# saber/ORB_SLAM2_Annotate

Measured on AMD Instinct MI355X. Metric: ORB extract+match frames/sec (kp/desc/matches bit-exact vs CPU oracle on the checked frames of every run), higher is better.
Workload: dtype u8; 1 GPU; KITTI 00 stereo 1241x376 nFeatures=2000: extract L+R + ComputeStereoMatches (synthetic stereo pairs; frames/s counts STEREO frames = 2 images each)

## Files before the change

orb_slam2_annotate_amd/csrc/k_match.hip:

```cpp
#include "kernels.h"
#include "match_kernels.h"

namespace orbfe {

namespace {
struct Desc { uint32_t w[8]; };

__device__ __forceinline__ Desc load_desc(const uint8_t* base, uint32_t idx) {
  const uint4* p = reinterpret_cast<const uint4*>(base + (size_t)idx * 32);
  const uint4 a = p[0], b = p[1];
  Desc d;
  d.w[0] = a.x; d.w[1] = a.y; d.w[2] = a.z; d.w[3] = a.w;
  d.w[4] = b.x; d.w[5] = b.y; d.w[6] = b.z; d.w[7] = b.w;
  return d;
}
__device__ __forceinline__ int hdist(const Desc& a, const Desc& b) {
  int d = 0;
#pragma unroll
  for (int i = 0; i < 8; i++) d += __popc(a.w[i] ^ b.w[i]);
  return d;
}
__device__ __forceinline__ uint32_t wave_min_u32(uint32_t v) { return wave_min_u32_dpp(v); }
__device__ __forceinline__ int rot_bin(float a1, float a2) {
  const float factor = 1.0f / 30;
// ... 236 lines not shown
    if (a.hasMp2[idx2]) continue;
    const bool st2 = a.stereo2[idx2] != 0;
    if (a.onlyStereo && !st2) continue;
    const uint32_t dist = (uint32_t)hdist(d1, load_desc(a.desc2, idx2));
    if (dist > 50u) continue;
    const float x2 = a.x2[idx2], y2 = a.y2[idx2];
    const int oc = a.octave2[idx2];
    if (!st1 && !st2) {
      const float dex = __fsub_rn(a.ex, x2), dey = __fsub_rn(a.ey, y2);
      if (__fadd_rn(__fmul_rn(dex, dex), __fmul_rn(dey, dey)) < __fmul_rn(100.0f, a.scaleFactors2[oc])) continue;
    }
    const float num = __fadd_rn(__fadd_rn(__fmul_rn(la, x2), __fmul_rn(lb, y2)), lc);
    if (den == 0) continue;
    const float dsqr = __fdiv_rn(__fmul_rn(num, num), den);
    if (!((double)dsqr < __dmul_rn(3.84, (double)a.levelSigma2_2[oc]))) continue;
    const uint32_t key = (dist << 16) | (0xffffu - (uint32_t)p);
    best = key < best ? key : best;
  }
  best = wave_min_u32(best);
  if (lane == 0) {
    if (best != 0xffffffffu) {
      const uint32_t pos = 0xffffu - (best & 0xffffu);
      const uint32_t idx2 = a.indices2[tq.off2 + pos];
      a.match[idx1] = (int32_t)idx2;
      a.bin[idx1] = (int8_t)rot_bin(a.angle1[idx1], a.angle2[idx2]);
    }
  }
}

__global__ __launch_bounds__(256) void k_search_triangulation(TriArgs a) {
  search_triangulation_one(a, blockIdx.x * 4 + (threadIdx.x >> 6), threadIdx.x & 63);
}
__global__ __launch_bounds__(256) void k_search_triangulation_multi(const TriArgs* __restrict__ args, const int32_t* __restrict__ blockStart,
                                                                    int K) {
  const int g = blockIdx.x;
  int lo = 0, hi = K;
  while (hi - lo > 1) {
    const int mid = (lo + hi) >> 1;
    if (blockStart[mid] <= g) lo = mid; else hi = mid;
  }
  const TriArgs a = args[lo];
  search_triangulation_one(a, (g - blockStart[lo]) * 4 + (threadIdx.x >> 6), threadIdx.x & 63);
}

__global__ __launch_bounds__(256) void k_rot_prune(int32_t* __restrict__ match, const int8_t* __restrict__ bin,
                                                   int n, int checkOri, int32_t* __restrict__ nMatches,
                                                   int batchStride) {
  match += (size_t)blockIdx.x * batchStride;
  bin += (size_t)blockIdx.x * batchStride;
  nMatches += blockIdx.x;
  __shared__ int hist[30];
  __shared__ int keep[3];
  __shared__ int total;
  const int tid = threadIdx.x;
  if (tid < 30) hist[tid] = 0;
  if (tid == 0) total = 0;
  __syncthreads();
  int mine = 0;
  for (int i = tid; i < n; i += 256)
    if (match[i] >= 0) { mine++; atomicAdd(&hist[bin[i]], 1); }
  if (mine) atomicAdd(&total, mine);
  __syncthreads();
  if (!checkOri) { if (tid == 0) *nMatches = total; return; }
  if (tid == 0) {
    int max1 = 0, max2 = 0, max3 = 0, i1 = -1, i2 = -1, i3 = -1;
    for (int i = 0; i < 30; i++) {
      const int s = hist[i];
      if (s > max1) { max3 = max2; max2 = max1; max1 = s; i3 = i2; i2 = i1; i1 = i; }
      else if (s > max2) { max3 = max2; max2 = s; i3 = i2; i2 = i; }
      else if (s > max3) { max3 = s; i3 = i; }
    }
    if ((float)max2 < __fmul_rn(0.1f, (float)max1)) { i2 = -1; i3 = -1; }
    else if ((float)max3 < __fmul_rn(0.1f, (float)max1)) { i3 = -1; }
    keep[0] = i1; keep[1] = i2; keep[2] = i3;
    int kept = 0;
    for (int i = 0; i < 30; i++)
      if (i == i1 || i == i2 || i == i3) kept += hist[i];
    *nMatches = kept;
  }
  __syncthreads();
  const int k0 = keep[0], k1 = keep[1], k2 = keep[2];
  for (int i = tid; i < n; i += 256)
    if (match[i] >= 0) {
      const int b = bin[i];
      if (b != k0 && b != k1 && b != k2) match[i] = -1;
    }
}

void launch_search_by_bow(hipStream_t s, const BowArgs& a, int nPairs, int maxCnt2) {
  if (nPairs <= 0) return;
  const size_t lds = (size_t)((maxCnt2 + 15) & ~15);
  if (maxCnt2 <= 64) hipLaunchKernelGGL((k_search_by_bow<1>), dim3(nPairs), dim3(64), lds, s, a);
  else if (maxCnt2 <= 128) hipLaunchKernelGGL((k_search_by_bow<2>), dim3(nPairs), dim3(64), lds, s, a);
  else hipLaunchKernelGGL((k_search_by_bow<4>), dim3(nPairs), dim3(64), lds, s, a);
}
void launch_search_by_bow_multi(hipStream_t s, const BowArgs* d_args, const int32_t* d_pairStart, int K, int nPairsTotal, int maxCnt2) {
  if (nPairsTotal <= 0 || K <= 0) return;
  const size_t lds = (size_t)((maxCnt2 + 15) & ~15);
  if (maxCnt2 <= 64) hipLaunchKernelGGL((k_search_by_bow_multi<1>), dim3(nPairsTotal), dim3(64), lds, s, d_args, d_pairStart, K);
  else if (maxCnt2 <= 128) hipLaunchKernelGGL((k_search_by_bow_multi<2>), dim3(nPairsTotal), dim3(64), lds, s, d_args, d_pairStart, K);
  else hipLaunchKernelGGL((k_search_by_bow_multi<4>), dim3(nPairsTotal), dim3(64), lds, s, d_args, d_pairStart, K);
}
void launch_search_triangulation(hipStream_t s, const TriArgs& a) {
  if (a.nQueries <= 0) return;
  hipLaunchKernelGGL(k_search_triangulation, dim3((a.nQueries + 3) / 4), dim3(256), 0, s, a);
}
void launch_search_triangulation_multi(hipStream_t s, const TriArgs* d_args, const int32_t* d_blockStart, int K, int totalBlocks) {
  if (K <= 0 || totalBlocks <= 0) return;
  hipLaunchKernelGGL(k_search_triangulation_multi, dim3(totalBlocks), dim3(256), 0, s, d_args, d_blockStart, K);
}
void launch_rot_prune(hipStream_t s, int32_t* match, const int8_t* bin, int n, int checkOri, int32_t* nMatches) {
  hipLaunchKernelGGL(k_rot_prune, dim3(1), dim3(256), 0, s, match, bin, n, checkOri, nMatches, 0);
}
void launch_rot_prune_batch(hipStream_t s, int32_t* match, const int8_t* bin, int n, int nArrays, int checkOri, int32_t* nMatches) {
  if (nArrays <= 0) return;
  hipLaunchKernelGGL(k_rot_prune, dim3(nArrays), dim3(256), 0, s, match, bin, n, checkOri, nMatches, n);
}
void launch_search_by_bow_batch(hipStream_t s, const BowBatch& b, int nPairs, int checkOri, int32_t* d_nMatches, int maxNodes) {
  if (nPairs <= 0 || b.capacity <= 0) return;
  const size_t lds = (size_t)((b.capacity + 15) & ~15);
  const int gx = (maxNodes > 0 && maxNodes < b.capacity) ? maxNodes : b.capacity;
  hipLaunchKernelGGL(k_search_by_bow_batch, dim3(gx, nPairs), dim3(64), lds, s, b);
  hipLaunchKernelGGL(k_rot_prune, dim3(nPairs), dim3(256), 0, s, b.match, b.bin, b.capacity, checkOri, d_nMatches,
                     b.capacity);
}

struct StereoPair {
  const float* kpL; const uint8_t* descL; int N;
  const float* kpR; const uint8_t* descR; int Nr;
  int frameL, frameR;
  float* uRight; float* depth; int32_t* sad;
  const int32_t* rowStart; const int32_t* sortedIdx; const float4* sortedRec;
};

__device__ __forceinline__ uint32_t row16_min_u32(uint32_t v) {
  uint32_t t;
  t = (uint32_t)__builtin_amdgcn_update_dpp((int)v, (int)v, 0x121, 0xf, 0xf, false); v = t < v ? t : v;
  t = (uint32_t)__builtin_amdgcn_update_dpp((int)v, (int)v, 0x122, 0xf, 0xf, false); v = t < v ? t : v;
  t = (uint32_t)__builtin_amdgcn_update_dpp((int)v, (int)v, 0x124, 0xf, 0xf, false); v = t < v ? t : v;
  t = (uint32_t)__builtin_amdgcn_update_dpp((int)v, (int)v, 0x128, 0xf, 0xf, false); v = t < v ? t : v;
  return v;
}
__device__ __forceinline__ int row16_sum_i32(int v) {
  v += __builtin_amdgcn_update_dpp(0, v, 0x121, 0xf, 0xf, false);
  v += __builtin_amdgcn_update_dpp(0, v, 0x122, 0xf, 0xf, false);
  v += __builtin_amdgcn_update_dpp(0, v, 0x124, 0xf, 0xf, false);
  v += __builtin_amdgcn_update_dpp(0, v, 0x128, 0xf, 0xf, false);
  return v;
}
constexpr uint32_t selpair(int o) { return (uint32_t)o | 0x0c00u | ((uint32_t)(o + 1) << 16) | 0x0c000000u; }

struct StereoLds { LevelView L[kMaxLevels], R[kMaxLevels]; float scale[2 * kMaxLevels]; };

template <bool kRec>
__device__ __forceinline__ void stereo_row16(const StereoArgs& a, const StereoLds& lv, const StereoPair& pp, int iL, bool alive,
                                             int lane) {
  const int sub = lane & 15, rowBase = lane & 48;
  float uL = 0.f, vL = 0.f;
  int levelL = 0;
  bool record = true;
  if (alive) {
    const float* kl = pp.kpL + (size_t)iL * 7;
    uL = kl[0]; vL = kl[1];
    levelL = reinterpret_cast<const int32_t*>(kl)[5];
    if ((unsigned)levelL >= (unsigned)a.pyrL.nlevels || !(fabsf(uL) < 3.0e38f) || !(fabsf(vL) < 3.0e38f)) { record = false; levelL = 0; uL = vL = 0.f; }
  }
  const int row = (int)vL;
  const float minU = __fsub_rn(uL, a.maxD), maxU = uL;
  bool live = alive && record && !(maxU < 0) && row >= 0 && row < a.rows;
  int pBeg = 0, pEnd = live ? pp.Nr : 0;
  if (pp.rowStart && live) {
    int band = a.bandR;
    {
      const int oMax = levelL + 1 < a.pyrL.nlevels ? levelL + 1 : a.pyrL.nlevels - 1;
      const int bl = (int)ceilf(__fmul_rn(2.0f, lv.scale[oMax < 0 ? 0 : oMax])) + 2;
      band = bl < band ? bl : band;
    }
    int lo = row - band, hi = row + band;
    lo = lo < 0 ? 0 : lo;
    hi = hi > a.rows - 1 ? a.rows - 1 : hi;
    if (lo > hi) { live = false; pEnd = 0; }
    else { pBeg = pp.rowStart[lo]; pEnd = pp.rowStart[hi + 1]; }
  }
  Desc dL = {};
  if (live) dL = load_desc(pp.descL, iL);
  uint32_t best = 0xffffffffu;
  float bestU = 0.f;
  for (int p = pBeg + sub; __any(p < pEnd); p += 16) {
    if (p < pEnd) {
      int iR, octR;
      float yR, uR;
      if (kRec) {
        const float4 rc = pp.sortedRec[p];
        uR = rc.x; yR = rc.y; octR = __float_as_int(rc.z); iR = __float_as_int(rc.w);
      } else {
        iR = pp.rowStart ? pp.sortedIdx[p] : p;
        const float* kr = pp.kpR + (size_t)iR * 7;
        octR = reinterpret_cast<const int32_t*>(kr)[5];
        yR = kr[1];
        uR = kr[0];
      }
      if ((unsigned)octR >= (unsigned)a.pyrL.nlevels || !(fabsf(yR) < 3.0e38f)) continue;
      const float r = __fmul_rn(2.0f, lv.scale[octR]);
      const int maxr = (int)ceilf(__fadd_rn(yR, r));
      const int minr = (int)floorf(__fsub_rn(yR, r));
      const bool cand = row >= minr && row <= maxr && octR >= levelL - 1 && octR <= levelL + 1 && uR >= minU && uR <= maxU;
      if (cand) {
        const uint32_t dist = (uint32_t)hdist(dL, load_desc(pp.descR, iR));
        const uint32_t key = (dist << 20) | (uint32_t)iR;
        if (dist < 100u && key < best) { best = key; bestU = uR; }
      }
    }
  }
  const uint32_t mine = best;
  best = row16_min_u32(best);
  live = live && best != 0xffffffffu && (int)(best >> 20) < 75;
  const unsigned long long win = __ballot(mine == best);
  const uint32_t winRow = (uint32_t)(win >> rowBase) & 0xffffu;
  const int src = rowBase + (winRow ? __builtin_ctz(winRow) : 0);
  const float uR0 = __shfl(bestU, src, 64);
  float oU = -1.0f, oD = -1.0f;
  int oS = -1;
  if (__builtin_amdgcn_ballot_w64(live) != 0ull) {
  const float sf = lv.scale[kMaxLevels + levelL];
  const float scaleduL = roundf(__fmul_rn(uL, sf));
  const float scaledvL = roundf(__fmul_rn(vL, sf));
  const float scaleduR0 = roundf(__fmul_rn(uR0, sf));
  const LevelView L = lv.L[levelL], R = lv.R[levelL];
  const float iniu = scaleduR0 + 5 - 5;
  const float endu = scaleduR0 + 5 + 5 + 1;
  if (iniu < 0 || endu >= (float)R.w) live = false;
  const int cy = (int)scaledvL, cxL = (int)scaleduL, cxR0 = (int)scaleduR0;
  if (cy < 5 || cy + 5 >= L.h || cy + 5 >= R.h || cxL < 5 || cxL + 5 >= L.w || cxR0 < 10) live = false;
  uint32_t ql[4] = {0u, 0u, 0u, 0u}, qr[6] = {0u, 0u, 0u, 0u, 0u, 0u};
  if (live && sub < 11) {
    const uint8_t* pl = L.base + (size_t)pp.frameL * L.frameStride + (ptrdiff_t)(cy + sub - 5) * L.pitch + (cxL - 5);
    const uint8_t* pr = R.base + (size_t)pp.frameR * R.frameStride + (ptrdiff_t)(cy + sub - 5) * R.pitch + (cxR0 - 10);
    struct __attribute__((packed, aligned(1))) U4u { uint32_t x, y, z, w; };
    struct __attribute__((packed, aligned(1))) U2u { uint32_t x, y; };
    const bool wide = cxL >= 5 && cxL + 10 < L.w && cxR0 >= 10 && cxR0 + 13 < R.w && cy >= 5 && cy + 5 < L.h && cy + 5 < R.h;
    if (wide) {
      const U4u a4 = *reinterpret_cast<const U4u*>(pl);
      const U4u b4 = *reinterpret_cast<const U4u*>(pr);
      const U2u c2 = *reinterpret_cast<const U2u*>(pr + 16);
      ql[0] = a4.x; ql[1] = a4.y; ql[2] = a4.z;
      qr[0] = b4.x; qr[1] = b4.y; qr[2] = b4.z; qr[3] = b4.w; qr[4] = c2.x; qr[5] = c2.y;
    } else {
#pragma unroll
      for (int k = 0; k < 11; k++) ql[k >> 2] |= (uint32_t)pl[k] << (8 * (k & 3));
#pragma unroll
      for (int k = 0; k < 21; k++) qr[k >> 2] |= (uint32_t)pr[k] << (8 * (k & 3));
    }
  }
  const uint32_t cL = ((uint32_t)__shfl((int)ql[1], rowBase + 5, 64) >> 8) & 0xffu;
  const uint32_t c1 = (uint32_t)__shfl((int)qr[1], rowBase + 5, 64), c2 = (uint32_t)__shfl((int)qr[2], rowBase + 5, 64),
                 c3 = (uint32_t)__shfl((int)qr[3], rowBase + 5, 64);
  const uint32_t cLL = cL | (cL << 16);
  uint32_t A[5], B[19], C[11];
#pragma unroll
  for (int m = 0; m < 5; m++) A[m] = __builtin_amdgcn_perm(ql[(m >> 1) + 1], ql[m >> 1], selpair((2 * m) & 3));
  const uint32_t l10 = (ql[2] >> 16) & 0xffu;
#pragma unroll
  for (int t = 0; t < 19; t++) B[t] = __builtin_amdgcn_perm(qr[(t >> 2) + 1], qr[t >> 2], selpair(t & 3)) + cLL;
#pragma unroll
  for (int t = 10; t < 21; t++) C[t - 10] = ((qr[t >> 2] >> (8 * (t & 3))) & 0xffu) + cL;
  int dists[11];
#pragma unroll
  for (int s = 0; s < 11; s++) {
    const int cb = 5 + s;
    const uint32_t cw = cb < 8 ? c1 : (cb < 12 ? c2 : c3);
    const uint32_t cR = (cw >> (8 * (cb & 3))) & 0xffu;
    const uint32_t cRR = cR | (cR << 16);
    uint32_t acc = 0;
#pragma unroll
    for (int m = 0; m < 5; m++) acc = __builtin_amdgcn_sad_u16(A[m] + cRR, B[2 * m + s], acc);
    acc = __builtin_amdgcn_sad_u16(l10 + cR, C[s], acc);
    dists[s] = row16_sum_i32(sub < 11 ? (int)acc : 0);
  }
  int bestSad = 0x7fffffff, bestinc = 0;
#pragma unroll
  for (int i = 0; i < 11; i++)
    if (dists[i] < bestSad) { bestSad = dists[i]; bestinc = i - 5; }
  if (bestinc == -5 || bestinc == 5) live = false;
  float d1 = 0, d2 = 0, d3 = 0;
#pragma unroll
  for (int i = 1; i < 10; i++)
    if (i == bestinc + 5) { d1 = (float)dists[i - 1]; d2 = (float)dists[i]; d3 = (float)dists[i + 1]; }
  const float deltaR = __fdiv_rn(__fsub_rn(d1, d3),
                                 __fmul_rn(2.0f, __fsub_rn(__fadd_rn(d1, d3), __fmul_rn(2.0f, d2))));
  if (deltaR < -1 || deltaR > 1) live = false;
  float bestuR = __fmul_rn(lv.scale[levelL], __fadd_rn(__fadd_rn(scaleduR0, (float)bestinc), deltaR));
  float disparity = __fsub_rn(uL, bestuR);
  if (live && disparity >= 0 && disparity < a.maxD) {
    if (disparity <= 0) {
      disparity = 0.01f;
      bestuR = (float)__dsub_rn((double)uL, 0.01);
    }
    oD = __fdiv_rn(a.mbf, disparity);
    oU = bestuR;
    oS = bestSad;
  }
  }
  if (alive && sub == 0) { pp.uRight[iL] = oU; pp.depth[iL] = oD; pp.sad[iL] = oS; }
}

__global__ __launch_bounds__(256) void k_stereo_bucket(const float* __restrict__ kpBase, const int32_t* __restrict__ nArr,
                                                       int nFixed, int capacity, int rows,
                                                       int32_t* __restrict__ rowStartBase,
                                                       int32_t* __restrict__ sortedBase, float4* __restrict__ recBase) {
  extern __shared__ int cnt[];
  __shared__ int waveTot[4];
  ORBFE_LATENCY_KERNEL_PRIO();
  const int tid = threadIdx.x, lane = tid & 63, wave = tid >> 6, p = blockIdx.x;
  const float* kpR = nArr ? kpBase + (size_t)(2 * p + 1) * capacity * 7 : kpBase;
  int Nr = nArr ? nArr[2 * p + 1] : nFixed;
  if (Nr > capacity) Nr = capacity;
  int32_t* rowStart = rowStartBase + (size_t)p * (rows + 1);
  int32_t* sorted = sortedBase + (size_t)p * capacity;
  float4* rec = recBase ? recBase + (size_t)p * capacity : nullptr;
  for (int i = tid; i <= rows; i += 256) cnt[i] = 0;
  __syncthreads();
  for (int i = tid; i < Nr; i += 256) {
    int b = (int)floorf(kpR[(size_t)i * 7 + 1]);
    b = b < 0 ? 0 : (b > rows - 1 ? rows - 1 : b);
    atomicAdd(&cnt[b], 1);
  }
  __syncthreads();
  int run = 0;
  for (int base = 0; base <= rows; base += 256) {
    const int i = base + tid;
    const int v = i <= rows ? cnt[i] : 0;
    int x = v;
#pragma unroll
    for (int o = 1; o < 64; o <<= 1) {
      const int y = __shfl_up(x, o, 64);
      if (lane >= o) x += y;
    }
    if (lane == 63) waveTot[wave] = x;
    __syncthreads();
    int b = run;
    for (int w = 0; w < wave; w++) b += waveTot[w];
    run += waveTot[0] + waveTot[1] + waveTot[2] + waveTot[3];
    if (i <= rows) { cnt[i] = b + x - v; rowStart[i] = b + x - v; }
    __syncthreads();
  }
  for (int i = tid; i < Nr; i += 256) {
    int b = (int)floorf(kpR[(size_t)i * 7 + 1]);
    b = b < 0 ? 0 : (b > rows - 1 ? rows - 1 : b);
    const int pos = atomicAdd(&cnt[b], 1);
    sorted[pos] = i;
    if (rec) rec[pos] = make_float4(kpR[(size_t)i * 7], kpR[(size_t)i * 7 + 1], __int_as_float(reinterpret_cast<const int32_t*>(kpR)[(size_t)i * 7 + 5]),
                                    __int_as_float(i));
  }
}

__device__ __forceinline__ void stereo_stage_views(const StereoArgs& a, StereoLds& lv) {
  const int t = threadIdx.x;
  if (t < kMaxLevels) lv.L[t] = a.pyrL.lv[t];
  else if (t < 2 * kMaxLevels) lv.R[t - kMaxLevels] = a.pyrR.lv[t - kMaxLevels];
  else if (t < 4 * kMaxLevels) lv.scale[t - 2 * kMaxLevels] = a.scaleTab[t - 2 * kMaxLevels];
  __syncthreads();
}

__global__ __launch_bounds__(256) void k_stereo_match(StereoArgs a) {
  __shared__ StereoLds lv;
  stereo_stage_views(a, lv);
  const int lane = threadIdx.x & 63;
  const int iL = blockIdx.x * 16 + (threadIdx.x >> 4);
  StereoPair pp = {a.kpL, a.descL, a.N, a.kpR, a.descR, a.Nr, a.frameL, a.frameR, a.uRight, a.depth, a.sad,
                   a.rowStart, a.sortedIdx, a.rowStart ? a.sortedRec : nullptr};
  if (pp.sortedRec) stereo_row16<true>(a, lv, pp, iL, iL < a.N, lane);
  else stereo_row16<false>(a, lv, pp, iL, iL < a.N, lane);
}

__global__ __launch_bounds__(256) void k_stereo_match_batch(const StereoArgs a, const StereoBatch b) {
  ORBFE_LATENCY_KERNEL_PRIO();
  __shared__ StereoLds lv;
  stereo_stage_views(a, lv);
  const int lane = threadIdx.x & 63;
  const int iL = blockIdx.x * 16 + (threadIdx.x >> 4);
  const int p = blockIdx.y;
  int N = b.n[2 * p], Nr = b.n[2 * p + 1];
  if (N > b.capacity) N = b.capacity;
  if (Nr > b.capacity) Nr = b.capacity;
  const size_t oL = (size_t)(2 * p) * b.capacity, oR = (size_t)(2 * p + 1) * b.capacity, oO = (size_t)p * b.capacity;
  if (iL < b.capacity && iL >= N && (lane & 15) == 0) {
    b.uRight[oO + iL] = -1.0f; b.depth[oO + iL] = -1.0f; b.sad[oO + iL] = -1;
  }
  if (blockIdx.x * 16 >= N) return;
  StereoPair pp;
  pp.kpL = b.kp + oL * 7; pp.descL = b.desc + oL * 32; pp.N = N;
  pp.kpR = b.kp + oR * 7; pp.descR = b.desc + oR * 32; pp.Nr = Nr;
  pp.frameL = 2 * p; pp.frameR = 2 * p + 1;
  pp.uRight = b.uRight + oO; pp.depth = b.depth + oO; pp.sad = b.sad + oO;
  pp.rowStart = a.rowStart ? a.rowStart + (size_t)p * (a.rows + 1) : nullptr;
  pp.sortedIdx = a.rowStart ? a.sortedIdx + (size_t)p * b.capacity : nullptr;
  pp.sortedRec = (a.rowStart && a.sortedRec) ? a.sortedRec + (size_t)p * b.capacity : nullptr;
  if (pp.sortedRec) stereo_row16<true>(a, lv, pp, iL, iL < N, lane);
  else stereo_row16<false>(a, lv, pp, iL, iL < N, lane);
}

__global__ __launch_bounds__(256) void k_stereo_median_cut(int N, const int32_t* __restrict__ sad,
                                                           float* __restrict__ uRight, float* __restrict__ depth,
                                                           int32_t* __restrict__ nStereo, int pairStride) {
  sad += (size_t)blockIdx.x * pairStride;
  uRight += (size_t)blockIdx.x * pairStride;
  depth += (size_t)blockIdx.x * pairStride;
  nStereo += blockIdx.x;
  __shared__ int hist[256];
  __shared__ int sel[3];
  __shared__ int waveTot[4];
  ORBFE_LATENCY_KERNEL_PRIO();
  const int tid = threadIdx.x;
  hist[tid] = 0;
  if (tid == 0) sel[2] = 0;
  __syncthreads();
  int mine = 0;
  for (int i = tid; i < N; i += 256) {
    const int s = sad[i];
    if (s >= 0) { atomicAdd(&hist[s >> 8], 1); mine++; }
  }
  if (mine) atomicAdd(&sel[2], mine);
  __syncthreads();
  const int total = sel[2];
  if (total == 0) { if (tid == 0) *nStereo = 0; return; }
  auto pick = [&](int k) {
    const int lane = tid & 63, wave = tid >> 6;
    const int v = hist[tid];
    int x = v;
#pragma unroll
    for (int o = 1; o < 64; o <<= 1) {
      const int y = __shfl_up(x, o, 64);
      if (lane >= o) x += y;
    }
    if (lane == 63) waveTot[wave] = x;
    __syncthreads();
    int base = 0;
    for (int w = 0; w < wave; w++) base += waveTot[w];
    const int incl = base + x;
    if (v > 0 && incl - v <= k && k < incl) { sel[0] = tid; sel[1] = k - (incl - v); }
    __syncthreads();
  };
  pick(total / 2);
  const int hi = sel[0];
  __syncthreads();
  hist[tid] = 0;
  __syncthreads();
  for (int i = tid; i < N; i += 256) {
    const int s = sad[i];
    if (s >= 0 && (s >> 8) == hi) atomicAdd(&hist[s & 255], 1);
  }
  __syncthreads();
  pick(sel[1]);
  const float median = (float)((hi << 8) | sel[0]);
  __syncthreads();
  if (tid == 0) sel[1] = 0;
  __syncthreads();
  const float thDist = __fmul_rn(1.5f * 1.4f, median);
  int kept = 0;
  for (int i = tid; i < N; i += 256) {
    const int s = sad[i];
    if (s < 0) continue;
    if ((float)s < thDist) kept++;
    else { uRight[i] = -1.0f; depth[i] = -1.0f; }
  }
  if (kept) atomicAdd(&sel[1], kept);
  __syncthreads();
  if (tid == 0) *nStereo = sel[1];
}

void launch_stereo(hipStream_t s, const StereoArgs& a, int32_t* d_nStereo) {
  if (a.N <= 0) return;
  if (a.rowStart)
    hipLaunchKernelGGL(k_stereo_bucket, dim3(1), dim3(256), (size_t)(a.rows + 1) * sizeof(int), s, a.kpR,
                       (const int32_t*)nullptr, a.Nr, a.Nr, a.rows, const_cast<int32_t*>(a.rowStart),
                       const_cast<int32_t*>(a.sortedIdx), const_cast<float4*>(a.sortedRec));
  hipLaunchKernelGGL(k_stereo_match, dim3((a.N + 15) / 16), dim3(256), 0, s, a);
  hipLaunchKernelGGL(k_stereo_median_cut, dim3(1), dim3(256), 0, s, a.N, a.sad, a.uRight, a.depth, d_nStereo, 0);
}

void launch_stereo_batch(hipStream_t s, const StereoArgs& a, const StereoBatch& b, int nPairs, int32_t* d_nStereo) {
  if (nPairs <= 0 || b.capacity <= 0) return;
  if (a.rowStart)
    hipLaunchKernelGGL(k_stereo_bucket, dim3(nPairs), dim3(256), (size_t)(a.rows + 1) * sizeof(int), s, b.kp, b.n, 0,
                       b.capacity, a.rows, const_cast<int32_t*>(a.rowStart), const_cast<int32_t*>(a.sortedIdx),
                       const_cast<float4*>(a.sortedRec));
  hipLaunchKernelGGL(k_stereo_match_batch, dim3((b.capacity + 15) / 16, nPairs), dim3(256), 0, s, a, b);
  hipLaunchKernelGGL(k_stereo_median_cut, dim3(nPairs), dim3(256), 0, s, b.capacity, b.sad, b.uRight, b.depth,
                     d_nStereo, b.capacity);
}

}
```

orb_slam2_annotate_amd/csrc/k_desc.hip:

```cpp
#include <cstdlib>

#include "kernels.h"

namespace orbfe {

namespace {
struct __attribute__((aligned(4))) U4 { uint32_t x, y, z, w; };
constexpr int kPatchRows = 37, kPatchDw = 12;

__device__ __forceinline__ int wave_sum(int x) {
  x += __builtin_amdgcn_update_dpp(0, x, 0x111, 0xf, 0xf, false);
  x += __builtin_amdgcn_update_dpp(0, x, 0x112, 0xf, 0xf, false);
  x += __builtin_amdgcn_update_dpp(0, x, 0x114, 0xf, 0xf, false);
  x += __builtin_amdgcn_update_dpp(0, x, 0x118, 0xf, 0xf, false);
  x += __builtin_amdgcn_update_dpp(0, x, 0x142, 0xa, 0xf, false);
  x += __builtin_amdgcn_update_dpp(0, x, 0x143, 0xc, 0xf, false);
  return __builtin_amdgcn_readlane(x, 63);
}
__device__ __forceinline__ void wave_sync_lds() {
  __builtin_amdgcn_fence(__ATOMIC_RELEASE, "wavefront");
  __builtin_amdgcn_wave_barrier();
  __builtin_amdgcn_fence(__ATOMIC_ACQUIRE, "wavefront");
}
}

template <int kKpPerBlock, int kUM, int kUD, bool kAbl>
__global__ __launch_bounds__(256) void k_orient_desc(OrientDescArgs a,
                                                     const LevelKp* __restrict__ levelKp,
                                                     const int32_t* __restrict__ levelCount,
                                                     const float4* __restrict__ patternF,
                                                     const uint4* __restrict__ momentTab,
                                                     const int32_t* __restrict__ umax,
                                                     float* __restrict__ kpOut,
                                                     uint8_t* __restrict__ descOut,
                                                     int32_t* __restrict__ nOut, int blocksPerFrame,
                                                     int nFrames, uint32_t blocksMagic,
                                                     int ablateArg ,
                                                     int interleave) {
  const int ablate = kAbl ? ablateArg : 0;
  __shared__ int s_m10[kKpPerBlock], s_m01[kKpPerBlock];
  __shared__ int s_x[kKpPerBlock], s_y[kKpPerBlock], s_level[kKpPerBlock], s_out[kKpPerBlock];
  __shared__ unsigned s_score[kKpPerBlock];
  __shared__ float s_angle[kKpPerBlock], s_cos[kKpPerBlock], s_sin[kKpPerBlock];
  __shared__ __attribute__((aligned(16))) uint32_t s_patch[4 * kUD * kPatchRows * kPatchDw];

  const int tid = threadIdx.x, lane = tid & 63, wave = tid >> 6;
  ORBFE_LATENCY_KERNEL_PRIO();
  const unsigned totalWork = (unsigned)blocksPerFrame * (unsigned)nFrames;
  const unsigned chunkW = (totalWork + 7u) >> 3;
  const unsigned perXcd = gridDim.x >> 3;
  for (unsigned itemInChunk = blockIdx.x >> 3; itemInChunk < chunkW; itemInChunk += perXcd) {
  const unsigned work = (blockIdx.x & 7u) * chunkW + itemInChunk;
  if (work >= totalWork) break;
  const int f = (int)udiv_magic(work, (uint32_t)blocksPerFrame, blocksMagic);
  const int slot0 = (int)(work - (unsigned)f * (unsigned)blocksPerFrame) * kKpPerBlock;
  const int32_t* cnt = levelCount + (size_t)f * a.nlevels;

  constexpr int kKpPerWave = kKpPerBlock / 4;
  const int myKp = wave * kKpPerWave + lane;
  if (lane < kKpPerWave) {
    const int slot = slot0 + (interleave ? wave + 4 * lane : myKp);
    int out = -1, l = 0;
    if (slot < a.kpSlotsPerFrame) {
      int base = 0;
      for (int k = 0; k < a.nlevels; k++) {
        if (slot >= a.kpStart[k]) { l = k; }
      }
      for (int k = 0; k < l; k++) base += cnt[k];
      const int i = slot - a.kpStart[l];
      if (i < cnt[l]) {
        const LevelKp kp = levelKp[(size_t)f * a.kpSlotsPerFrame + slot];
        if (base + (int)kp.rank < a.outCapacity) out = base + (int)kp.rank;
        s_x[myKp] = kp.x;
        s_y[myKp] = kp.y;
        s_score[myKp] = kp.score;
      }
    }
    s_level[myKp] = l;
    s_out[myKp] = out;
    if (slot == 0) {
      int tot = 0;
      for (int k = 0; k < a.nlevels; k++) tot += cnt[k];
      nOut[f] = tot;
    }
  }
  wave_sync_lds();

  {
    const int row = lane >> 1, half = lane & 1;
    const int dy = row - 15;
    const int ady = dy < 0 ? -dy : dy;
    const bool active = row < 31;
    uint4 wt = make_uint4(0, 0, 0, 0), mk = make_uint4(0, 0, 0, 0);
    if (active) {
      const int d = umax[ady];
      wt = momentTab[(d * 2 + half) * 2];
      mk = momentTab[(d * 2 + half) * 2 + 1];
    }
    for (int j0 = wave * kKpPerWave; j0 < wave * kKpPerWave + kKpPerWave; j0 += kUM) {
      uint32_t dw[kUM][4];
      int kout[kUM];
#pragma unroll
      for (int u = 0; u < kUM; u++) {
        const int j = j0 + u;
#pragma unroll
        for (int k = 0; k < 4; k++) dw[u][k] = 0;
        kout[u] = __builtin_amdgcn_readfirstlane(s_out[j]);
        if (kout[u] >= 0) {
          const int kl = __builtin_amdgcn_readfirstlane(s_level[j]);
          const int kx = __builtin_amdgcn_readfirstlane(s_x[j]), ky = __builtin_amdgcn_readfirstlane(s_y[j]);
          const LevelView lv = a.pyr.lv[kl];
          const uint8_t* origin = lv.base + (size_t)f * lv.frameStride + (size_t)(ky - 15) * lv.pitch + (kx - 15);
          if (active && !(ablate & 1)) {
            const uint8_t* p = origin + (uint32_t)(row * lv.pitch + (half ? 16 : 0));
            {
              struct __attribute__((packed, aligned(1))) U4u { uint32_t x, y, z, w; };
              const U4u q = *reinterpret_cast<const U4u*>(p);
              dw[u][0] = q.x; dw[u][1] = q.y; dw[u][2] = q.z; dw[u][3] = q.w;
            }
          }
        }
      }
#pragma unroll
      for (int u = 0; u < kUM; u++) {
        const int j = j0 + u;
        if (kout[u] < 0) continue;
        const uint32_t q0 = dw[u][0], q1 = dw[u][1], q2 = dw[u][2], q3 = dw[u][3];
        unsigned w = __builtin_amdgcn_udot4(q0, wt.x, 0u, false);
        w = __builtin_amdgcn_udot4(q1, wt.y, w, false);
        w = __builtin_amdgcn_udot4(q2, wt.z, w, false);
        w = __builtin_amdgcn_udot4(q3, wt.w, w, false);
        unsigned sm = __builtin_amdgcn_udot4(q0, mk.x, 0u, false);
        sm = __builtin_amdgcn_udot4(q1, mk.y, sm, false);
        sm = __builtin_amdgcn_udot4(q2, mk.z, sm, false);
        sm = __builtin_amdgcn_udot4(q3, mk.w, sm, false);
        const int sW = (int)w - 16 * (int)sm;
        const int sI = dy * (int)sm;
        const int m10 = wave_sum(sW), m01 = wave_sum(sI);
        if (lane == 0) { s_m10[j] = m10; s_m01[j] = m01; }
      }
    }
  }
  wave_sync_lds();

  if (lane < kKpPerWave && s_out[myKp] >= 0) {
    const float angle = fast_atan2((float)s_m01[myKp], (float)s_m10[myKp]);
    const float factorPI = (float)(3.1415926535897932384626433832795 / 180.f);
    float ca, sb;
    sincos_spec(__fmul_rn(angle, factorPI), &ca, &sb);
    s_angle[myKp] = angle;
    s_cos[myKp] = ca;
    s_sin[myKp] = sb;
  }
  wave_sync_lds();

  {
    float4 P[4];
#pragma unroll
    for (int j = 0; j < 4; j++) P[j] = patternF[lane + 64 * j];
    uint32_t* myPatch = &s_patch[wave * kUD * kPatchRows * kPatchDw];
    constexpr int kKpPerWave3 = kKpPerBlock / 4;
    const int jBeg = wave * kKpPerWave3, jEnd = jBeg + kKpPerWave3;
    U4 stage[kUD][2];
    int colOffN[kUD], koutN[kUD];
    auto request = [&](int j0) {
#pragma unroll
      for (int u = 0; u < kUD; u++) {
        const int j = j0 + u;
        colOffN[u] = 0;
        koutN[u] = __builtin_amdgcn_readfirstlane(s_out[j]);
        if (koutN[u] < 0) continue;
        const int kl = __builtin_amdgcn_readfirstlane(s_level[j]);
        const int kx = __builtin_amdgcn_readfirstlane(s_x[j]), ky = __builtin_amdgcn_readfirstlane(s_y[j]);
        const LevelView bl = a.blur.lv[kl];
        int ws = (kx - 18) & ~3;
        if (ws > bl.pitch - 4 * kPatchDw) ws = bl.pitch - 4 * kPatchDw;
        colOffN[u] = kx - ws;
        const uint8_t* pb = bl.base + (size_t)f * bl.frameStride + (size_t)(ky - 18) * bl.pitch + ws;
#pragma unroll
        for (int h = 0; h < 2; h++) {
          const int idx = lane + 64 * h;
          const int row = (idx * 43) >> 7, part = idx - 3 * row;
          if (idx < 3 * kPatchRows && !(ablate & 2)) stage[u][h] = *reinterpret_cast<const U4*>(pb + (uint32_t)(row * bl.pitch + 16 * part));
          else stage[u][h] = U4{0u, 0u, 0u, 0u};
        }
      }
    };
#ifdef ORBFE_DESC_PIPELINE
    request(jBeg);
#endif
    for (int j0 = jBeg; j0 < jEnd; j0 += kUD) {
#ifndef ORBFE_DESC_PIPELINE
      request(j0);
#endif
      int t0v[kUD][4], t1v[kUD][4];
      int colOff[kUD], kout[kUD];
#pragma unroll
      for (int u = 0; u < kUD; u++) {
        colOff[u] = colOffN[u];
        kout[u] = koutN[u];
        if (kout[u] < 0) continue;
#pragma unroll
        for (int h = 0; h < 2; h++) {
          const int idx = lane + 64 * h;
          if (idx < 3 * kPatchRows)
            *reinterpret_cast<uint4*>(&myPatch[u * kPatchRows * kPatchDw + 4 * idx]) =
                make_uint4(stage[u][h].x, stage[u][h].y, stage[u][h].z, stage[u][h].w);
        }
      }
#ifdef ORBFE_DESC_PIPELINE
      if (j0 + kUD < jEnd) request(j0 + kUD);
#endif
      __builtin_amdgcn_fence(__ATOMIC_RELEASE, "wavefront");
      __builtin_amdgcn_wave_barrier();
      __builtin_amdgcn_fence(__ATOMIC_ACQUIRE, "wavefront");
#pragma unroll
      for (int u = 0; u < kUD; u++) {
        const int j = j0 + u;
        if (kout[u] < 0) continue;
        const float ca = s_cos[j], sb = s_sin[j];
        const uint8_t* pbytes = reinterpret_cast<const uint8_t*>(s_patch);
        constexpr float kMagic = 12582912.0f;
        constexpr uint32_t kBias = 0x4B400000u * 49u;
        const uint32_t baseK = (uint32_t)((wave * kUD + u) * kPatchRows * kPatchDw * 4 + 18 * 4 * kPatchDw + colOff[u]) - kBias;
#pragma unroll
        for (int t = 0; t < 4; t++) {
          const float x0 = P[t].x, x1 = P[t].y, y0 = P[t].z, y1 = P[t].w;
          const float r0 = __fadd_rn(__fadd_rn(__fmul_rn(x0, sb), __fmul_rn(y0, ca)), kMagic);
          const float r1 = __fadd_rn(__fadd_rn(__fmul_rn(x1, sb), __fmul_rn(y1, ca)), kMagic);
          const float c0 = __fadd_rn(__fsub_rn(__fmul_rn(x0, ca), __fmul_rn(y0, sb)), kMagic);
          const float c1 = __fadd_rn(__fsub_rn(__fmul_rn(x1, ca), __fmul_rn(y1, sb)), kMagic);
          const uint32_t ir0 = __float_as_uint(r0), ir1 = __float_as_uint(r1);
          const uint32_t ic0 = __float_as_uint(c0), ic1 = __float_as_uint(c1);
          t0v[u][t] = (ablate & 4) ? (int)(ir0 & 255u) : pbytes[baseK + ir0 * (4u * kPatchDw) + ic0];
          t1v[u][t] = (ablate & 4) ? (int)(ic1 & 255u) : pbytes[baseK + ir1 * (4u * kPatchDw) + ic1];
        }
      }
      __builtin_amdgcn_fence(__ATOMIC_RELEASE, "wavefront");
      __builtin_amdgcn_wave_barrier();
#pragma unroll
      for (int u = 0; u < kUD; u++) {
        const int j = j0 + u;
        const int outIdx = kout[u];
        if (outIdx < 0) continue;
        unsigned long long* dout = reinterpret_cast<unsigned long long*>(
            descOut + ((size_t)f * a.outCapacity + outIdx) * 32);
        uint32_t bitsLo = 0, bitsHi = 0;
#pragma unroll
        for (int t = 0; t < 4; t++) {
          const unsigned long long bt = __ballot(t0v[u][t] < t1v[u][t]);
          bitsLo = lane == t ? (uint32_t)bt : bitsLo;
          bitsHi = lane == t ? (uint32_t)(bt >> 32) : bitsHi;
        }
        if (lane < 4) dout[lane] = (unsigned long long)bitsLo | ((unsigned long long)bitsHi << 32);
        {
          const int l = __builtin_amdgcn_readfirstlane(s_level[j]);
          const float sc = a.scale[l];
          const uint32_t wx = __float_as_uint(__fmul_rn((float)s_x[j], sc)), wy = __float_as_uint(__fmul_rn((float)s_y[j], sc));
          const uint32_t wa = __float_as_uint(s_angle[j]), ws = __float_as_uint((float)s_score[j]);
          const uint32_t wz = __float_as_uint(a.kpSize[l]);
          uint32_t w = 0xffffffffu;
          w = lane == 5 ? (uint32_t)l : w;
          w = lane == 4 ? ws : w;
          w = lane == 3 ? wa : w;
          w = lane == 2 ? wz : w;
          w = lane == 1 ? wy : w;
          w = lane == 0 ? wx : w;
          if (lane < 7) reinterpret_cast<uint32_t*>(kpOut + ((size_t)f * a.outCapacity + outIdx) * 7)[lane] = w;
        }
      }
    }
  }
  wave_sync_lds();
  }
}

#ifndef ORBFE_ORIENT_UM
#define ORBFE_ORIENT_UM 4
#endif
#ifndef ORBFE_ORIENT_UD
#define ORBFE_ORIENT_UD 2
#endif

void launch_orient_desc(hipStream_t s, const OrientDescArgs& a, const LevelKp* d_levelKp,
                        const int32_t* d_levelCount, const float4* d_patternF, const uint4* d_momentTab,
                        const int32_t* d_umax, int nFrames, void* d_kpOut, uint8_t* d_descOut,
                        int32_t* d_nOut, int concurrentLaunches) {
  if (nFrames <= 0 || a.kpSlotsPerFrame <= 0) return;
  const bool latencyForm = nFrames <= 8;
  static const int kKpbEnv = getenv("ORBFE_ORIENT_KPB") ? atoi(getenv("ORBFE_ORIENT_KPB")) : 64;
  const int kpb = latencyForm ? 16 : (kKpbEnv == 256 ? 256 : (kKpbEnv == 128 ? 128 : 64));
  const int blocksPerFrame = (a.kpSlotsPerFrame + kpb - 1) / kpb;
  const unsigned total = (unsigned)blocksPerFrame * (unsigned)nFrames;
  const uint32_t blocksMagic = udiv_magic_multiplier((uint32_t)blocksPerFrame);
  static const size_t kPad = occupancy_pad_bytes("ORIENT", 0);
  static const int kGridEnv = getenv("ORBFE_ORIENT_GRID") ? atoi(getenv("ORBFE_ORIENT_GRID")) : -1;
  int kGridPerCu = kGridEnv;
  if (kGridPerCu < 0) {
    kGridPerCu = 16 / (concurrentLaunches < 1 ? 1 : concurrentLaunches);
    kGridPerCu = kGridPerCu < 2 ? 2 : (kGridPerCu > 4 ? 4 : kGridPerCu);
    if (a.kpSlotsPerFrame >= 24 * 64 && concurrentLaunches >= 8) kGridPerCu = 1;
    if (concurrentLaunches <= 1) kGridPerCu = 0;
  }
  const unsigned full = (total + 7u) / 8u * 8u;
  static const int kAblate = getenv("ORBFE_ORIENT_ABLATE") ? atoi(getenv("ORBFE_ORIENT_ABLATE")) : 0;
  static const int kInterleave = getenv("ORBFE_ORIENT_INTERLEAVE") ? atoi(getenv("ORBFE_ORIENT_INTERLEAVE")) : 1;
  if (latencyForm) {
    if (kAblate)
      hipLaunchKernelGGL((k_orient_desc<16, ORBFE_ORIENT_UM, ORBFE_ORIENT_UD, true>), dim3(full), dim3(256), 0, s, a, d_levelKp, d_levelCount,
                         d_patternF, d_momentTab, d_umax, (float*)d_kpOut, d_descOut, d_nOut, blocksPerFrame, nFrames, blocksMagic, kAblate, kInterleave);
    else
      hipLaunchKernelGGL((k_orient_desc<16, ORBFE_ORIENT_UM, ORBFE_ORIENT_UD, false>), dim3(full), dim3(256), 0, s, a, d_levelKp, d_levelCount,
                         d_patternF, d_momentTab, d_umax, (float*)d_kpOut, d_descOut, d_nOut, blocksPerFrame, nFrames, blocksMagic, 0, kInterleave);
  } else {
    unsigned grid = full;
    if (kGridPerCu > 0 && (unsigned)kGridPerCu * 256u < full) grid = (unsigned)kGridPerCu * 256u;
#define ORBFE_LAUNCH_ORIENT(KPB, ABL)                                                                                      \
  hipLaunchKernelGGL((k_orient_desc<KPB, ORBFE_ORIENT_UM, ORBFE_ORIENT_UD, ABL>), dim3(grid), dim3(256), kPad, s, a, d_levelKp, d_levelCount, d_patternF, \
                     d_momentTab, d_umax, (float*)d_kpOut, d_descOut, d_nOut, blocksPerFrame, nFrames, blocksMagic, kAblate, kInterleave)
    if (kAblate) ORBFE_LAUNCH_ORIENT(64, true);
    else if (kpb == 256) ORBFE_LAUNCH_ORIENT(256, false);
    else if (kpb == 128) ORBFE_LAUNCH_ORIENT(128, false);
    else ORBFE_LAUNCH_ORIENT(64, false);
#undef ORBFE_LAUNCH_ORIENT
  }
}

void build_moment_table(uint8_t* tab ) {
  for (int d = 0; d < 16; d++)
    for (int half = 0; half < 2; half++)
      for (int i = 0; i < 16; i++) {
        const int dx = half ? i + 1 : i - 15;
        const int adx = dx < 0 ? -dx : dx;
        const bool in = adx <= d && adx <= 15;
        tab[((d * 2 + half) * 2 + 0) * 16 + i] = (uint8_t)(in ? dx + 16 : 0);
        tab[((d * 2 + half) * 2 + 1) * 16 + i] = (uint8_t)(in ? 1 : 0);
      }
}

}
```

Before: 108,300 stereo frames/s.

## Compact live stereo candidates in LDS before SAD refinement in batch kernel

The stereo match is split into a descriptor search phase and a SAD refinement phase. In the batched kernel, each block now handles 64 left keypoints. Surviving candidates are compacted into a shared-memory list, and waves then run the expensive patch refinement only on dense groups of live candidates. This targets wave divergence, where refinement previously ran with many idle 16-lane rows, at the cost of an extra block barrier, LDS traffic, fewer blocks and possible load imbalance.

```diff
diff --git a/orb_slam2_annotate_amd/csrc/k_match.hip b/orb_slam2_annotate_amd/csrc/k_match.hip
--- a/orb_slam2_annotate_amd/csrc/k_match.hip
+++ b/orb_slam2_annotate_amd/csrc/k_match.hip
@@ -412,9 +412,11 @@
 
 struct StereoLds { LevelView L[kMaxLevels], R[kMaxLevels]; float scale[2 * kMaxLevels]; };
 
+struct StereoCand { int iL, levelL; float uL, vL, uR0; };
+
 template <bool kRec>
-__device__ __forceinline__ void stereo_row16(const StereoArgs& a, const StereoLds& lv, const StereoPair& pp, int iL, bool alive,
-                                             int lane) {
+__device__ __forceinline__ bool stereo_search16(const StereoArgs& a, const StereoLds& lv, const StereoPair& pp, int iL, bool alive,
+                                                int lane, StereoCand& c) {
   const int sub = lane & 15, rowBase = lane & 48;
   float uL = 0.f, vL = 0.f;
   int levelL = 0;
@@ -478,7 +480,17 @@
   const unsigned long long win = __ballot(mine == best);
   const uint32_t winRow = (uint32_t)(win >> rowBase) & 0xffffu;
   const int src = rowBase + (winRow ? __builtin_ctz(winRow) : 0);
-  const float uR0 = __shfl(bestU, src, 64);
+  c.iL = iL; c.levelL = levelL; c.uL = uL; c.vL = vL;
+  c.uR0 = __shfl(bestU, src, 64);
+  return live;
+}
+
+__device__ __forceinline__ void stereo_refine16(const StereoArgs& a, const StereoLds& lv, const StereoPair& pp, const StereoCand& c,
+                                                bool valid, int lane) {
+  const int sub = lane & 15, rowBase = lane & 48;
+  const int iL = c.iL, levelL = c.levelL;
+  const float uL = c.uL, vL = c.vL, uR0 = c.uR0;
+  bool live = valid;
   float oU = -1.0f, oD = -1.0f;
   int oS = -1;
   if (__builtin_amdgcn_ballot_w64(live) != 0ull) {
@@ -561,7 +573,10 @@
     oS = bestSad;
   }
   }
-  if (alive && sub == 0) { pp.uRight[iL] = oU; pp.depth[iL] = oD; pp.sad[iL] = oS; }
+  if (valid && sub == 0) { pp.uRight[iL] = oU; pp.depth[iL] = oD; pp.sad[iL] = oS; }
+}
+__device__ __forceinline__ void stereo_store_none(const StereoPair& pp, int iL) {
+  pp.uRight[iL] = -1.0f; pp.depth[iL] = -1.0f; pp.sad[iL] = -1;
 }
 
 __global__ __launch_bounds__(256) void k_stereo_bucket(const float* __restrict__ kpBase, const int32_t* __restrict__ nArr,
@@ -629,25 +644,38 @@
   const int iL = blockIdx.x * 16 + (threadIdx.x >> 4);
   StereoPair pp = {a.kpL, a.descL, a.N, a.kpR, a.descR, a.Nr, a.frameL, a.frameR, a.uRight, a.depth, a.sad,
                    a.rowStart, a.sortedIdx, a.rowStart ? a.sortedRec : nullptr};
-  if (pp.sortedRec) stereo_row16<true>(a, lv, pp, iL, iL < a.N, lane);
-  else stereo_row16<false>(a, lv, pp, iL, iL < a.N, lane);
-}
-
+  const bool alive = iL < a.N;
+  StereoCand c;
+  const bool live = pp.sortedRec ? stereo_search16<true>(a, lv, pp, iL, alive, lane, c)
+                                 : stereo_search16<false>(a, lv, pp, iL, alive, lane, c);
+  if (alive && !live && (lane & 15) == 0) stereo_store_none(pp, iL);
+  stereo_refine16(a, lv, pp, c, live, lane);
+}
+
+#ifndef ORBFE_STEREO_G
+#define ORBFE_STEREO_G 64
+#endif
+constexpr int kStereoG = ORBFE_STEREO_G;
+static_assert(kStereoG % 64 == 0, "a wave takes kStereoG / 4 left keypoints, four per round");
 __global__ __launch_bounds__(256) void k_stereo_match_batch(const StereoArgs a, const StereoBatch b) {
   ORBFE_LATENCY_KERNEL_PRIO();
   __shared__ StereoLds lv;
+  __shared__ StereoCand list[kStereoG];
+  __shared__ int listN[4];
   stereo_stage_views(a, lv);
-  const int lane = threadIdx.x & 63;
-  const int iL = blockIdx.x * 16 + (threadIdx.x >> 4);
+  const int lane = threadIdx.x & 63, sub = lane & 15, q = lane >> 4;
+  const int wave = __builtin_amdgcn_readfirstlane(threadIdx.x >> 6);
+  const int base = blockIdx.x * kStereoG;
   const int p = blockIdx.y;
   int N = b.n[2 * p], Nr = b.n[2 * p + 1];
   if (N > b.capacity) N = b.capacity;
   if (Nr > b.capacity) Nr = b.capacity;
   const size_t oL = (size_t)(2 * p) * b.capacity, oR = (size_t)(2 * p + 1) * b.capacity, oO = (size_t)p * b.capacity;
-  if (iL < b.capacity && iL >= N && (lane & 15) == 0) {
-    b.uRight[oO + iL] = -1.0f; b.depth[oO + iL] = -1.0f; b.sad[oO + iL] = -1;
-  }
-  if (blockIdx.x * 16 >= N) return;
+  for (int i = threadIdx.x; i < kStereoG; i += 256) {
+    const int iL = base + i;
+    if (iL < b.capacity && iL >= N) { b.uRight[oO + iL] = -1.0f; b.depth[oO + iL] = -1.0f; b.sad[oO + iL] = -1; }
+  }
+  if (base >= N) return;
   StereoPair pp;
   pp.kpL = b.kp + oL * 7; pp.descL = b.desc + oL * 32; pp.N = N;
   pp.kpR = b.kp + oR * 7; pp.descR = b.desc + oR * 32; pp.Nr = Nr;
@@ -656,8 +684,38 @@
   pp.rowStart = a.rowStart ? a.rowStart + (size_t)p * (a.rows + 1) : nullptr;
   pp.sortedIdx = a.rowStart ? a.sortedIdx + (size_t)p * b.capacity : nullptr;
   pp.sortedRec = (a.rowStart && a.sortedRec) ? a.sortedRec + (size_t)p * b.capacity : nullptr;
-  if (pp.sortedRec) stereo_row16<true>(a, lv, pp, iL, iL < N, lane);
-  else stereo_row16<false>(a, lv, pp, iL, iL < N, lane);
+  constexpr int kSeg = kStereoG / 4;
+  int nMine = 0;
+#pragma unroll 1
+  for (int r = 0; r < kSeg / 4; r++) {
+    const int iL = base + wave * kSeg + r * 4 + q;
+    const bool alive = iL < N;
+    StereoCand c;
+    const bool live = pp.sortedRec ? stereo_search16<true>(a, lv, pp, iL, alive, lane, c)
+                                   : stereo_search16<false>(a, lv, pp, iL, alive, lane, c);
+    const unsigned long long heads = __builtin_amdgcn_ballot_w64(live) & 0x0001000100010001ull;
+    if (sub == 0) {
+      if (live) list[wave * kSeg + nMine + __popcll(heads & ((1ull << (lane & 48)) - 1ull))] = c;
+      else if (alive) stereo_store_none(pp, iL);
+    }
+    nMine += __popcll(heads);
+  }
+  if (lane == 0) listN[wave] = nMine;
+  __syncthreads();
+  const int n0 = __builtin_amdgcn_readfirstlane(listN[0]), n1 = __builtin_amdgcn_readfirstlane(listN[1]),
+            n2 = __builtin_amdgcn_readfirstlane(listN[2]), n3 = __builtin_amdgcn_readfirstlane(listN[3]);
+  const int total = n0 + n1 + n2 + n3;
+#pragma unroll 1
+  for (int e0 = wave * 4; e0 < total; e0 += 16) {
+    const int e = e0 + q;
+    const bool valid = e < total;
+    StereoCand c = {0, 0, 0.f, 0.f, 0.f};
+    if (valid) {
+      const int slot = e < n0 ? e : (e < n0 + n1 ? kSeg + e - n0 : (e < n0 + n1 + n2 ? 2 * kSeg + e - n0 - n1 : 3 * kSeg + e - n0 - n1 - n2));
+      c = list[slot];
+    }
+    stereo_refine16(a, lv, pp, c, valid, lane);
+  }
 }
 
 __global__ __launch_bounds__(256) void k_stereo_median_cut(int N, const int32_t* __restrict__ sad,
@@ -745,7 +803,7 @@
     hipLaunchKernelGGL(k_stereo_bucket, dim3(nPairs), dim3(256), (size_t)(a.rows + 1) * sizeof(int), s, b.kp, b.n, 0,
                        b.capacity, a.rows, const_cast<int32_t*>(a.rowStart), const_cast<int32_t*>(a.sortedIdx),
                        const_cast<float4*>(a.sortedRec));
-  hipLaunchKernelGGL(k_stereo_match_batch, dim3((b.capacity + 15) / 16, nPairs), dim3(256), 0, s, a, b);
+  hipLaunchKernelGGL(k_stereo_match_batch, dim3((b.capacity + kStereoG - 1) / kStereoG, nPairs), dim3(256), 0, s, a, b);
   hipLaunchKernelGGL(k_stereo_median_cut, dim3(nPairs), dim3(256), 0, s, b.capacity, b.sad, b.uRight, b.depth,
                      d_nStereo, b.capacity);
 }
```

Result: slower. 105,900 stereo frames/s (-2.2%).

## Batch moment reductions across keypoints with permlane/DPP transpose-fold and pack LDS keypoint fields

Applied to the files above, without the earlier changes.

Replaces the per-keypoint full-wave DPP reduction of the orientation moments with a batched transpose-style reduction. It uses permlane32/permlane16 swaps and DPP folds so each lane ends up holding one keypoint's m10/m01. The angle is then computed straight from registers, which removes the s_m10/s_m01 LDS round trip and one wave sync. Keypoint x/y are packed into one word and out-index and level into another, cutting LDS arrays and readfirstlane reads. The cost is more register pressure from holding up to 16 partials, plus reliance on gfx950 permlane swap instructions.

```diff
diff --git a/orb_slam2_annotate_amd/csrc/k_desc.hip b/orb_slam2_annotate_amd/csrc/k_desc.hip
--- a/orb_slam2_annotate_amd/csrc/k_desc.hip
+++ b/orb_slam2_annotate_amd/csrc/k_desc.hip
@@ -1,6 +1,7 @@
 #include <cstdlib>
 
 #include "kernels.h"
+#include "moment_reduce.h"
 
 namespace orbfe {
 
@@ -8,15 +9,6 @@
 struct __attribute__((aligned(4))) U4 { uint32_t x, y, z, w; };
 constexpr int kPatchRows = 37, kPatchDw = 12;
 
-__device__ __forceinline__ int wave_sum(int x) {
-  x += __builtin_amdgcn_update_dpp(0, x, 0x111, 0xf, 0xf, false);
-  x += __builtin_amdgcn_update_dpp(0, x, 0x112, 0xf, 0xf, false);
-  x += __builtin_amdgcn_update_dpp(0, x, 0x114, 0xf, 0xf, false);
-  x += __builtin_amdgcn_update_dpp(0, x, 0x118, 0xf, 0xf, false);
-  x += __builtin_amdgcn_update_dpp(0, x, 0x142, 0xa, 0xf, false);
-  x += __builtin_amdgcn_update_dpp(0, x, 0x143, 0xc, 0xf, false);
-  return __builtin_amdgcn_readlane(x, 63);
-}
 __device__ __forceinline__ void wave_sync_lds() {
   __builtin_amdgcn_fence(__ATOMIC_RELEASE, "wavefront");
   __builtin_amdgcn_wave_barrier();
@@ -38,8 +30,8 @@
                                                      int ablateArg ,
                                                      int interleave) {
   const int ablate = kAbl ? ablateArg : 0;
-  __shared__ int s_m10[kKpPerBlock], s_m01[kKpPerBlock];
-  __shared__ int s_x[kKpPerBlock], s_y[kKpPerBlock], s_level[kKpPerBlock], s_out[kKpPerBlock];
+  __shared__ int s_ol[kKpPerBlock];
+  __shared__ unsigned s_xy[kKpPerBlock];
   __shared__ unsigned s_score[kKpPerBlock];
   __shared__ float s_angle[kKpPerBlock], s_cos[kKpPerBlock], s_sin[kKpPerBlock];
   __shared__ __attribute__((aligned(16))) uint32_t s_patch[4 * kUD * kPatchRows * kPatchDw];
@@ -61,31 +53,33 @@
   if (lane < kKpPerWave) {
     const int slot = slot0 + (interleave ? wave + 4 * lane : myKp);
     int out = -1, l = 0;
+    int base = 0, start = 0, n = 0, tot = 0;
+    for (int k = 0; k < a.nlevels; k++) {
+      const int c = cnt[k];
+      if (slot >= a.kpStart[k]) { l = k; start = a.kpStart[k]; n = c; base = tot; }
+      tot += c;
+    }
     if (slot < a.kpSlotsPerFrame) {
-      int base = 0;
-      for (int k = 0; k < a.nlevels; k++) {
-        if (slot >= a.kpStart[k]) { l = k; }
-      }
-      for (int k = 0; k < l; k++) base += cnt[k];
-      const int i = slot - a.kpStart[l];
-      if (i < cnt[l]) {
+      const int i = slot - start;
+      if (i < n) {
         const LevelKp kp = levelKp[(size_t)f * a.kpSlotsPerFrame + slot];
         if (base + (int)kp.rank < a.outCapacity) out = base + (int)kp.rank;
-        s_x[myKp] = kp.x;
-        s_y[myKp] = kp.y;
+        s_xy[myKp] = (unsigned)kp.x | ((unsigned)kp.y << 16);
         s_score[myKp] = kp.score;
       }
     }
-    s_level[myKp] = l;
-    s_out[myKp] = out;
-    if (slot == 0) {
-      int tot = 0;
-      for (int k = 0; k < a.nlevels; k++) tot += cnt[k];
-      nOut[f] = tot;
-    }
+    s_ol[myKp] = out * 16 + l;
+    if (slot == 0) nOut[f] = tot;
   }
   wave_sync_lds();
 
+  constexpr int kKC = kKpPerWave < 16 ? kKpPerWave : 16, kChunks = kKpPerWave / kKC;
+  constexpr int kG = kUM < kKC ? kUM : kKC;
+  constexpr int kLanesPerKp = 32 / kKC;
+  static_assert(kKC % kG == 0 && kChunks <= 2 * kLanesPerKp, "chunking of the moment reduction");
+  const int dup = (lane & (kLanesPerKp - 1)) + kLanesPerKp * (lane >> 5);
+  const int kp2 = wave * kKpPerWave + dup * kKC + (lane & 31) / kLanesPerKp;
+  int m10 = 0, m01 = 0;
   {
     const int row = lane >> 1, half = lane & 1;
     const int dy = row - 15;
@@ -97,18 +91,23 @@
       wt = momentTab[(d * 2 + half) * 2];
       mk = momentTab[(d * 2 + half) * 2 + 1];
     }
-    for (int j0 = wave * kKpPerWave; j0 < wave * kKpPerWave + kKpPerWave; j0 += kUM) {
-      uint32_t dw[kUM][4];
-      int kout[kUM];
-#pragma unroll
-      for (int u = 0; u < kUM; u++) {
+#pragma unroll 1
+    for (int c = 0; c < kChunks; c++) {
+    int part[kKC];
+#pragma unroll
+    for (int g = 0; g < kKC; g += kG) {
+      const int j0 = wave * kKpPerWave + c * kKC + g;
+      uint32_t dw[kG][4];
+      int kout[kG];
+#pragma unroll
+      for (int u = 0; u < kG; u++) {
         const int j = j0 + u;
 #pragma unroll
         for (int k = 0; k < 4; k++) dw[u][k] = 0;
-        kout[u] = __builtin_amdgcn_readfirstlane(s_out[j]);
+        kout[u] = __builtin_amdgcn_readfirstlane(s_ol[j]);
+        const unsigned kxy = __builtin_amdgcn_readfirstlane(s_xy[j]);
         if (kout[u] >= 0) {
-          const int kl = __builtin_amdgcn_readfirstlane(s_level[j]);
-          const int kx = __builtin_amdgcn_readfirstlane(s_x[j]), ky = __builtin_amdgcn_readfirstlane(s_y[j]);
+          const int kl = kout[u] & 15, kx = (int)(kxy & 0xffffu), ky = (int)(kxy >> 16);
           const LevelView lv = a.pyr.lv[kl];
           const uint8_t* origin = lv.base + (size_t)f * lv.frameStride + (size_t)(ky - 15) * lv.pitch + (kx - 15);
           if (active && !(ablate & 1)) {
@@ -122,9 +121,7 @@
         }
       }
 #pragma unroll
-      for (int u = 0; u < kUM; u++) {
-        const int j = j0 + u;
-        if (kout[u] < 0) continue;
+      for (int u = 0; u < kG; u++) {
         const uint32_t q0 = dw[u][0], q1 = dw[u][1], q2 = dw[u][2], q3 = dw[u][3];
         unsigned w = __builtin_amdgcn_udot4(q0, wt.x, 0u, false);
         w = __builtin_amdgcn_udot4(q1, wt.y, w, false);
@@ -136,21 +133,24 @@
         sm = __builtin_amdgcn_udot4(q3, mk.w, sm, false);
         const int sW = (int)w - 16 * (int)sm;
         const int sI = dy * (int)sm;
-        const int m10 = wave_sum(sW), m01 = wave_sum(sI);
-        if (lane == 0) { s_m10[j] = m10; s_m01[j] = m01; }
-      }
-    }
-  }
-  wave_sync_lds();
-
-  if (lane < kKpPerWave && s_out[myKp] >= 0) {
-    const float angle = fast_atan2((float)s_m01[myKp], (float)s_m10[myKp]);
+        part[g + u] = fold_halves(sW, sI);
+        asm volatile("" : "+v"(part[g + u]));
+      }
+    }
+    int t10, t01;
+    moments_to_lanes<kKC>(part, lane, t10, t01);
+    if (dup == c) { m10 = t10; m01 = t01; }
+    }
+  }
+
+  if (dup < kChunks && s_ol[kp2] >= 0) {
+    const float angle = fast_atan2((float)m01, (float)m10);
     const float factorPI = (float)(3.1415926535897932384626433832795 / 180.f);
     float ca, sb;
     sincos_spec(__fmul_rn(angle, factorPI), &ca, &sb);
-    s_angle[myKp] = angle;
-    s_cos[myKp] = ca;
-    s_sin[myKp] = sb;
+    s_angle[kp2] = angle;
+    s_cos[kp2] = ca;
+    s_sin[kp2] = sb;
   }
   wave_sync_lds();
 
@@ -163,15 +163,16 @@
     const int jBeg = wave * kKpPerWave3, jEnd = jBeg + kKpPerWave3;
     U4 stage[kUD][2];
     int colOffN[kUD], koutN[kUD];
+    unsigned kxyN[kUD];
     auto request = [&](int j0) {
 #pragma unroll
       for (int u = 0; u < kUD; u++) {
         const int j = j0 + u;
         colOffN[u] = 0;
-        koutN[u] = __builtin_amdgcn_readfirstlane(s_out[j]);
+        koutN[u] = __builtin_amdgcn_readfirstlane(s_ol[j]);
+        kxyN[u] = __builtin_amdgcn_readfirstlane(s_xy[j]);
         if (koutN[u] < 0) continue;
-        const int kl = __builtin_amdgcn_readfirstlane(s_level[j]);
-        const int kx = __builtin_amdgcn_readfirstlane(s_x[j]), ky = __builtin_amdgcn_readfirstlane(s_y[j]);
+        const int kl = koutN[u] & 15, kx = (int)(kxyN[u] & 0xffffu), ky = (int)(kxyN[u] >> 16);
         const LevelView bl = a.blur.lv[kl];
         int ws = (kx - 18) & ~3;
         if (ws > bl.pitch - 4 * kPatchDw) ws = bl.pitch - 4 * kPatchDw;
@@ -195,10 +196,12 @@
 #endif
       int t0v[kUD][4], t1v[kUD][4];
       int colOff[kUD], kout[kUD];
+      unsigned kxy[kUD];
 #pragma unroll
       for (int u = 0; u < kUD; u++) {
         colOff[u] = colOffN[u];
         kout[u] = koutN[u];
+        kxy[u] = kxyN[u];
         if (kout[u] < 0) continue;
 #pragma unroll
         for (int h = 0; h < 2; h++) {
@@ -241,8 +244,8 @@
 #pragma unroll
       for (int u = 0; u < kUD; u++) {
         const int j = j0 + u;
-        const int outIdx = kout[u];
-        if (outIdx < 0) continue;
+        if (kout[u] < 0) continue;
+        const int outIdx = kout[u] >> 4;
         unsigned long long* dout = reinterpret_cast<unsigned long long*>(
             descOut + ((size_t)f * a.outCapacity + outIdx) * 32);
         uint32_t bitsLo = 0, bitsHi = 0;
@@ -254,9 +257,10 @@
         }
         if (lane < 4) dout[lane] = (unsigned long long)bitsLo | ((unsigned long long)bitsHi << 32);
         {
-          const int l = __builtin_amdgcn_readfirstlane(s_level[j]);
+          const int l = kout[u] & 15;
           const float sc = a.scale[l];
-          const uint32_t wx = __float_as_uint(__fmul_rn((float)s_x[j], sc)), wy = __float_as_uint(__fmul_rn((float)s_y[j], sc));
+          const uint32_t wx = __float_as_uint(__fmul_rn((float)(int)(kxy[u] & 0xffffu), sc));
+          const uint32_t wy = __float_as_uint(__fmul_rn((float)(int)(kxy[u] >> 16), sc));
           const uint32_t wa = __float_as_uint(s_angle[j]), ws = __float_as_uint((float)s_score[j]);
           const uint32_t wz = __float_as_uint(a.kpSize[l]);
           uint32_t w = 0xffffffffu;
diff --git a/orb_slam2_annotate_amd/csrc/moment_reduce.h b/orb_slam2_annotate_amd/csrc/moment_reduce.h
--- /dev/null
+++ b/orb_slam2_annotate_amd/csrc/moment_reduce.h
@@ -0,0 +1,47 @@
+#pragma once
+
+namespace orbfe {
+
+template <int kCtrl>
+__device__ __forceinline__ int dpp_mov(int x) { return __builtin_amdgcn_update_dpp(0, x, kCtrl, 0xf, 0xf, false); }
+constexpr int kDppXor1 = 0xB1 , kDppXor2 = 0x4E ;
+constexpr int kDppRor8 = 0x128 , kDppHalfMirror = 0x141 ;
+template <int kCtrl, int kHalf>
+__device__ __forceinline__ void fold_dpp(int* r, bool upper) {
+#pragma unroll
+  for (int i = 0; i < kHalf; i++) {
+    const int keep = upper ? r[i + kHalf] : r[i], send = upper ? r[i] : r[i + kHalf];
+    r[i] = keep + dpp_mov<kCtrl>(send);
+  }
+}
+__device__ __forceinline__ int fold_halves(int sw, int si) {
+  const auto p = __builtin_amdgcn_permlane32_swap((unsigned)sw, (unsigned)si, false, false);
+  return (int)(p[0] + p[1]);
+}
+template <int kKC>
+__device__ __forceinline__ void moments_to_lanes(const int* c, int lane, int& m10, int& m01) {
+  static_assert(kKC == 4 || kKC == 16, "the row levels below are written for 2 and 8 registers per row");
+  constexpr int R = kKC / 2;
+  int d[R];
+#pragma unroll
+  for (int k = 0; k < R; k++) {
+    const auto p = __builtin_amdgcn_permlane16_swap((unsigned)c[k], (unsigned)c[k + R], false, false);
+    d[k] = (int)(p[0] + p[1]);
+  }
+  int t;
+  if constexpr (R == 8) {
+    fold_dpp<kDppRor8, 4>(d, (lane & 8) != 0);
+    fold_dpp<kDppHalfMirror, 2>(d, (lane & 4) != 0);
+    fold_dpp<kDppXor2, 1>(d, (lane & 2) != 0);
+    t = d[0] + dpp_mov<kDppXor1>(d[0]);
+  } else {
+    fold_dpp<kDppRor8, 1>(d, (lane & 8) != 0);
+    t = d[0] + dpp_mov<kDppHalfMirror>(d[0]);
+    t += dpp_mov<kDppXor1>(t);
+    t += dpp_mov<kDppXor2>(t);
+  }
+  const auto p = __builtin_amdgcn_permlane32_swap((unsigned)t, (unsigned)t, false, false);
+  m10 = (int)p[0];
+  m01 = (int)p[1];
+}
+}
```

New measurement: 105,100 stereo frames/s before, 105,900 stereo frames/s after, median of 6. About the same (+0.8%).
